# laurentbartholdi/SpaSM.jl

Measured on AMD Instinct MI355X. Metric: Schur nnz reduced/sec (GF(p) echelonize), 1Mx1M CSR, higher is better.
Workload: dtype int32 (GF(p) balanced residues); 1 GPU; BASELINE config 3: 1000000x1000000 CSR, 20 nnz/row, p=65521, seed 0x5A5A0003, Schur round 0; rows_per_gpu=1000000, npiv=169473, nnz_out=522630694, parallelism=single GPU

## Files before the change

### spasm.jl_amd/csrc/engine.hip

```cpp
#include "common.hpp"
#include "kernels.hpp"
#include "stream.hpp"
#include "wlevel.hpp"
#include "greedy.hpp"
#include "dense.hpp"
#include "spmv.hpp"
#include "spgemm.hpp"
#include "reshape.hpp"
#include "trsolve.hpp"
#include "batch.hpp"
#include "blocks.hpp"
#include "solve_batch.hpp"
#include "solver.hpp"
#include <cstring>
#include <rocprim/device/device_scan.hpp>
#include <rocprim/device/device_radix_sort.hpp>
#include <rocprim/device/device_segmented_radix_sort.hpp>
#include <vector>
#include <memory>
#include <stdexcept>
#include <type_traits>
#include <algorithm>
#include <cstring>
#include <cstdlib>
// ... 163 lines not shown
    default: break;
    }
}

template <int LOGT, int TPR, int WPB, int B, bool SMALL, int MINW = 1, int EPL = 1, int QX = 0, bool BLOOM = false, bool SEG = false> void launch_wstream(const StreamArgs &a, int nrows, int num_cu, size_t lds, hipStream_t s)
{
    static int per_cu_dev[kMaxDev] = {0};
    int &per_cu = per_cu_dev[current_device()];
    if (!per_cu) {
        HIPCHK(hipFuncSetAttribute((const void *)k_wstream<LOGT, TPR, WPB, B, SMALL, MINW, EPL, QX, BLOOM, SEG>, hipFuncAttributeMaxDynamicSharedMemorySize, (int)lds));
        int nb = 0;
        HIPCHK(hipOccupancyMaxActiveBlocksPerMultiprocessor(&nb, (const void *)k_wstream<LOGT, TPR, WPB, B, SMALL, MINW, EPL, QX, BLOOM, SEG>, WPB * 64, lds));
        per_cu = std::max(nb, 1);
    }
    if (nrows <= 0) return;
    const int rows_per_block = TPR == 64 ? WPB : 1;
    const int grid = std::max(1, std::min((nrows + rows_per_block - 1) / rows_per_block, num_cu * per_cu));
    hipLaunchKernelGGL((k_wstream<LOGT, TPR, WPB, B, SMALL, MINW, EPL, QX, BLOOM, SEG>), dim3(grid), dim3(WPB * 64), lds, s, a);
    HIPCHK(hipGetLastError());
}

inline bool stream_bloom()
{
    const char *e = getenv("SPASM_AMD_BLOOM");
    return e && atoi(e) != 0;
}
inline int stream_chunk_log()
{
    const char *e = getenv("SPASM_AMD_CHUNK");
    return e && atoi(e) == 128 ? 7 : 6;
}
enum StreamMode { STREAM_SEG = 0, STREAM_CHUNK64 = 1, STREAM_BLOOM = 2, STREAM_CHUNK128 = 3 };
inline StreamMode stream_mode(i64 buffer_entries)
{
    if (stream_chunk_log() == 7) return STREAM_CHUNK128;
    if (stream_bloom()) return STREAM_BLOOM;
    return buffer_entries < ((i64)1 << 29) ? STREAM_SEG : STREAM_CHUNK64;
}

const int kNumStreamClasses = 7;
inline int stream_logt(int c) { return 8 + c; }
inline int stream_tpr(int c) { return c <= 2 ? 64 : (c == 3 ? 128 : 256); }
inline int stream_wpb(int c) { return c == 3 ? 2 : 4; }
template <bool SMALL> void launch_stream_class(int cls, const StreamArgs &a, int nrows, int num_cu, size_t lds, hipStream_t s, StreamMode mode)
{
    if (mode == STREAM_SEG) {
        switch (cls) {
        case 0: launch_wstream<8, 64, 4, 4, SMALL, 1, 1, 0, false, true>(a, nrows, num_cu, lds, s); break;
        case 1: launch_wstream<9, 64, 4, 8, SMALL, 1, 1, 0, false, true>(a, nrows, num_cu, lds, s); break;
        case 2: launch_wstream<10, 64, 4, 8, SMALL, 1, 1, 0, false, true>(a, nrows, num_cu, lds, s); break;
        case 3: launch_wstream<11, 128, 2, 8, SMALL, 1, 1, 0, false, true>(a, nrows, num_cu, lds, s); break;
        case 4: launch_wstream<12, 256, 4, 8, SMALL, 1, 1, 0, false, true>(a, nrows, num_cu, lds, s); break;
        case 5: launch_wstream<13, 256, 4, 8, SMALL, 1, 1, 0, false, true>(a, nrows, num_cu, lds, s); break;
        case 6: launch_wstream<14, 256, 4, 8, SMALL, 1, 1, 0, false, true>(a, nrows, num_cu, lds, s); break;
        default: break;
        }
        return;
    }
    if (mode == STREAM_CHUNK128) {
        switch (cls) {
        case 0: launch_wstream<8, 64, 4, 2, SMALL, 1, 2>(a, nrows, num_cu, lds, s); break;
        case 1: launch_wstream<9, 64, 4, 4, SMALL, 1, 2>(a, nrows, num_cu, lds, s); break;
        case 2: launch_wstream<10, 64, 4, 4, SMALL, 1, 2>(a, nrows, num_cu, lds, s); break;
        case 3: launch_wstream<11, 128, 2, 4, SMALL, 1, 2>(a, nrows, num_cu, lds, s); break;
        case 4: launch_wstream<12, 256, 4, 4, SMALL, 1, 2>(a, nrows, num_cu, lds, s); break;
        case 5: launch_wstream<13, 256, 4, 4, SMALL, 1, 2>(a, nrows, num_cu, lds, s); break;
        case 6: launch_wstream<14, 256, 4, 4, SMALL, 1, 2>(a, nrows, num_cu, lds, s); break;
        default: break;
        }
        return;
    }
    if (mode == STREAM_BLOOM) {
        switch (cls) {
        case 0: launch_wstream<8, 64, 4, 4, SMALL, 1, 1, 0, true>(a, nrows, num_cu, lds, s); break;
        case 1: launch_wstream<9, 64, 4, 8, SMALL, 1, 1, 0, true>(a, nrows, num_cu, lds, s); break;
        case 2: launch_wstream<10, 64, 4, 8, SMALL, 1, 1, 0, true>(a, nrows, num_cu, lds, s); break;
        case 3: launch_wstream<11, 128, 2, 8, SMALL, 1, 1, 0, true>(a, nrows, num_cu, lds, s); break;
        case 4: launch_wstream<12, 256, 4, 8, SMALL, 1, 1, 0, true>(a, nrows, num_cu, lds, s); break;
        case 5: launch_wstream<13, 256, 4, 8, SMALL, 1, 1, 0, true>(a, nrows, num_cu, lds, s); break;
        case 6: launch_wstream<14, 256, 4, 8, SMALL, 1, 1, 0, true>(a, nrows, num_cu, lds, s); break;
        default: break;
        }
        return;
    }
    switch (cls) {
    case 0: launch_wstream<8, 64, 4, 4, SMALL>(a, nrows, num_cu, lds, s); break;
    case 1: launch_wstream<9, 64, 4, 8, SMALL>(a, nrows, num_cu, lds, s); break;
    case 2: launch_wstream<10, 64, 4, 8, SMALL>(a, nrows, num_cu, lds, s); break;
    case 3: launch_wstream<11, 128, 2, 8, SMALL>(a, nrows, num_cu, lds, s); break;
    case 4: launch_wstream<12, 256, 4, 8, SMALL>(a, nrows, num_cu, lds, s); break;
    case 5: launch_wstream<13, 256, 4, 8, SMALL>(a, nrows, num_cu, lds, s); break;
    case 6: launch_wstream<14, 256, 4, 8, SMALL>(a, nrows, num_cu, lds, s); break;
    default: break;
    }
}

struct Round {
    ZpField F;
    int m = 0;
    int num_cu = 256;
    hipStream_t stream = nullptr;
    Scanner scan;

    DevBuf<u64d> best;
    DevBuf<int> colflag, colscan, qinv_r, pivrow, pivcol, is_piv, rowflag, rowscan, np_rows;
    int npiv = 0, nnp = 0;
    DevBuf<i64d> ulen, uoff;
    i64 utotal = 0;
    DevBuf<int2> Ufull, UPP, UPN;
    DevBuf<UHdr> uhdr;
    bool use_uinv = false;
    DevMat E;
    DevBuf<int2> UinvPool;
    DevBuf<i64d> UinvStart, ubound;
    DevBuf<int> UinvLen;
    DevBuf<int4> colinfo;
    DevBuf<unsigned> pbits;
    DevBuf<i64d> rstart;
    DevBuf<int> rlen;
    i64 uinv_nnz = 0;
    DevBuf<int4> Lpool;
    DevBuf<int> Lidx;
    bool want_idx = false;
    DevBuf<int> sflag;
    DevBuf<int2> fixbuf;
    DevBuf<int> fixcnt;
    bool use_stream = true;
    StreamMode smode = STREAM_SEG;
    bool use_w = false;
    bool force_lists = false;
    DevBuf<int4> wcol;
    DevBuf<int2> wrow;
    DevBuf<int> wreject_list;
    i64 wtotal = 0;
    i64 wcap = 0;
    i64 w_entries = 0, w_long_rows = 0;
    i64 own_base = 0, wbase = 0;
    i64 own_total = 0;
    DevBuf<u64d> own_ctr;
    DevBuf<u64d> wstate, wblk;
    DevBuf<int> wmid_list, wbig_list, wbig_count;
    std::vector<int> wbig_at;
    bool want_w_row_stats = false;
    DevBuf<WLevRec> lev_recs;
    DevBuf<unsigned> lev0_sz, lev0_off;
    DevBuf<u64d> lev0_ent;
    i64 lev0_total = 0, lev0_entries = 0;
    int wave_per_cu_blocks = 0;
    DevBuf<int> lev, lev_keys, lev_iota, lev_order, lev_start_d, lev_flag;
    DevBuf<unsigned char> sort_tmp;
    std::vector<int> lev_start;
    int depth = -1;
    bool quiet_rejects = false;
    DevBuf<u64d> pool_ctr;
    int npool_active = NPOOL;
    u64d region_cap = 0;
    DevBuf<i64d> Lstart, bound, sstart;
    DevBuf<int> Llen, overflow_list, overflow2_list, fail_list;
    DevBuf<long long> pmask;
    int big_blocks = 0, big_npiv = -1;
    DevBuf<int> xdense;
    DevBuf<unsigned> bitmap;
    DevBuf<int4> bigscratch;
    DevBuf<RoundCounters> ctr;
    RoundCounters hctr;
    DevBuf<int> class_count, class_list;
    DevBuf<RowDesc> class_desc;
    int bigsc_blocks = 0, bigsc_m = -1;
    DevBuf<long long> sc_xdense;
    DevBuf<unsigned> sc_bitmap;
    DevBuf<int> sc_touched;
    DevBuf<u64d> stamps;
    DevMat S;
    i64 s_capacity = 0;
    i64 s_total_bound = 0;
    int free_cols = 0;
    hipEvent_t ev[5] = {nullptr, nullptr, nullptr, nullptr, nullptr};
    hipStream_t side = nullptr;
    hipStream_t twin_s[3] = {nullptr, nullptr, nullptr};
    hipEvent_t twin_ev[3] = {nullptr, nullptr, nullptr};
    hipEvent_t ev_fork = nullptr, ev_join = nullptr;
    hipStream_t lane_s[4] = {nullptr, nullptr, nullptr, nullptr};
    hipEvent_t lane_ev[4] = {nullptr, nullptr, nullptr, nullptr};
    hipEvent_t ev_cls_done[NHASHMAX] = {nullptr, nullptr, nullptr, nullptr, nullptr, nullptr, nullptr, nullptr};
    hipEvent_t ev_cls[NCLASS + 1];
    int launch_cls[NCLASS];
    int nlaunch = 0;
    int hclass_count[NCLASS];
    int nhash_used = 0;
    bool class_timing = true;

    Round()
    {
        memset(&hctr, 0, sizeof hctr);
        for (auto &e : ev) HIPCHK(hipEventCreate(&e));
        for (auto &e : ev_cls) { e = nullptr; HIPCHK(hipEventCreate(&e)); }
        memset(hclass_count, 0, sizeof hclass_count);
        memset(launch_cls, 0, sizeof launch_cls);
        if (const char *e = getenv("SPASM_AMD_STREAM")) use_stream = atoi(e) != 0;
        int dev = 0;
        hipDeviceProp_t prop;
        if (hipGetDevice(&dev) == hipSuccess && hipGetDeviceProperties(&prop, dev) == hipSuccess) num_cu = prop.multiProcessorCount;
    }
    ~Round()
    {
        for (auto &e : ev) if (e) (void)hipEventDestroy(e);
        for (auto &e : ev_cls) if (e) (void)hipEventDestroy(e);
        for (auto &e : ev_w) if (e) (void)hipEventDestroy(e);
        if (ev_fork) (void)hipEventDestroy(ev_fork);
        if (ev_join) (void)hipEventDestroy(ev_join);
        for (auto &e : lane_ev) if (e) (void)hipEventDestroy(e);
        for (auto &l : lane_s) if (l) (void)hipStreamDestroy(l);
        for (auto &e : ev_cls_done) if (e) (void)hipEventDestroy(e);
        if (side) (void)hipStreamDestroy(side);
        for (auto &e : twin_ev) if (e) (void)hipEventDestroy(e);
        for (auto &l : twin_s) if (l) (void)hipStreamDestroy(l);
    }

    void elect_local(const DevMat &A, int row_base, int row_stride = 1)
    {
        m = A.m;
        best.ensure((size_t)m + 1);
        hipLaunchKernelGGL(k_fill_u64, dim3(cdiv((i64)m + 1, 256)), dim3(256), 0, stream, (i64d)m + 1, (u64d)NO_BEST, best.p);
        HIPCHK(hipGetLastError());
        if (A.n > 0) {
            hipLaunchKernelGGL(k_elect, dim3(cdiv(A.n, 256)), dim3(256), 0, stream, A.n, row_base, row_stride, A.len.p, A.lead.p, best.p);
            HIPCHK(hipGetLastError());
        }
    }

    void assign_pivots()
    {
        colflag.ensure((size_t)m + 1);
        colscan.ensure((size_t)m + 1);
        qinv_r.ensure((size_t)m + 1);
        hipLaunchKernelGGL(k_col_flags, dim3(cdiv((i64)m + 1, 256)), dim3(256), 0, stream, m, best.p, colflag.p);
        HIPCHK(hipGetLastError());
        scan.exclusive(colflag.p, colscan.p, (size_t)m + 1, stream);
        HIPCHK(hipMemcpyAsync(&npiv, colscan.p + m, sizeof(int), hipMemcpyDeviceToHost, stream));
        HIPCHK(hipStreamSynchronize(stream));
        pivrow.ensure((size_t)npiv + 1);
        pivcol.ensure((size_t)npiv + 1);
        if (m > 0) {
            hipLaunchKernelGGL(k_col_assign, dim3(cdiv(m, 256)), dim3(256), 0, stream, m, best.p, colscan.p, qinv_r.p, pivrow.p, pivcol.p);
            HIPCHK(hipGetLastError());
        }
    }

    DevBuf<int> closed, colcnt, prop, newflag, newscan;
    bool quiet_fallbacks = false;
    bool quiet_known = false;
    DevBuf<int> pivval;
    bool want_pivval = false;
    DevBuf<u64d> best2;
    int n_leftmost = 0, n_open = 0;
    DevBuf<int> newpass, newidx, newrow_of_col, newrows;
    int open_count[OPEN_PASSES + 1] = {0};
    int open_nnew = 0, open_npass = 0;
    void open_begin(const DevMat &A, int row_base, int row_stride)
    {
        n_leftmost = npiv;
        n_open = 0;
        open_nnew = open_npass = 0;
        for (int &c : open_count) c = 0;
        closed.ensure((size_t)m + 1); colcnt.ensure((size_t)m + 1); newflag.ensure((size_t)m + 1); newscan.ensure((size_t)m + 1);
        newpass.ensure((size_t)m + 1); newidx.ensure((size_t)m + 1); newrow_of_col.ensure((size_t)m + 1); newrows.ensure((size_t)m + 1);
        best2.ensure((size_t)m + 1);
        prop.ensure((size_t)A.n + 1);
        is_piv.ensure((size_t)A.n + 1);
        HIPCHK(hipMemsetAsync(closed.p, 0, ((size_t)m + 1) * sizeof(int), stream));
        HIPCHK(hipMemsetAsync(newpass.p, 0, ((size_t)m + 1) * sizeof(int), stream));
        HIPCHK(hipMemsetAsync(is_piv.p, 0, ((size_t)A.n + 1) * sizeof(int), stream));
        if (npiv > 0) {
            hipLaunchKernelGGL(k_mark_rows, dim3(cdiv(npiv, 256)), dim3(256), 0, stream, npiv, row_base, row_stride, A.n, pivrow.p, is_piv.p);
            constexpr int TEAM = 8;
            hipLaunchKernelGGL((k_close_cols<TEAM>), dim3(cdiv((i64)npiv * TEAM, 256)), dim3(256), 0, stream, npiv, pivrow.p, row_base, row_stride, A.n, A.start.p, A.len.p,
                               A.ent.p, closed.p);
            HIPCHK(hipGetLastError());
        }
    }
    void open_hist(const DevMat &A)
    {
        HIPCHK(hipMemsetAsync(colcnt.p, 0, ((size_t)m + 1) * sizeof(int), stream));
        HIPCHK(hipMemsetAsync(newflag.p, 0, ((size_t)m + 1) * sizeof(int), stream));
        hipLaunchKernelGGL(k_fill_u64, dim3(cdiv((i64)m + 1, 256)), dim3(256), 0, stream, (i64d)m + 1, (u64d)NO_BEST, best2.p);
        if (A.n > 0) hipLaunchKernelGGL(k_col_histogram, dim3(cdiv((i64)A.n * 8, 256)), dim3(256), 0, stream, A.n, is_piv.p, A.start.p, A.len.p, A.ent.p, colcnt.p);
        HIPCHK(hipGetLastError());
    }
    void open_propose(const DevMat &A, int row_base, int row_stride)
    {
        constexpr int TEAM = 8;
        if (A.n > 0)
            hipLaunchKernelGGL((k_propose_open<TEAM>), dim3(cdiv((i64)A.n * TEAM, 256)), dim3(256), 0, stream, A.n, row_base, row_stride, is_piv.p, A.start.p, A.len.p,
                               A.ent.p, closed.p, colcnt.p, prop.p, best2.p);
        HIPCHK(hipGetLastError());
    }
    void open_accept(const DevMat &A, int row_base, int row_stride)
    {
        constexpr int TEAM = 8;
        if (A.n > 0)
            hipLaunchKernelGGL((k_accept_open<TEAM>), dim3(cdiv((i64)A.n * TEAM, 256)), dim3(256), 0, stream, A.n, row_base, row_stride, A.start.p, A.len.p, A.ent.p,
                               prop.p, best2.p, newflag.p);
        HIPCHK(hipGetLastError());
    }
    int open_record(const DevMat &A, int pass, int row_base, int row_stride)
    {
        scan.exclusive(newflag.p, newscan.p, (size_t)m + 1, stream);
        int nacc = 0;
        HIPCHK(hipMemcpyAsync(&nacc, newscan.p + m, sizeof(int), hipMemcpyDeviceToHost, stream));
        HIPCHK(hipStreamSynchronize(stream));
        if (nacc == 0) return 0;
        constexpr int TEAM = 8;
        hipLaunchKernelGGL(k_record_open, dim3(cdiv(m, 256)), dim3(256), 0, stream, m, pass, newflag.p, newscan.p, best2.p, newpass.p, newidx.p,
                           newrow_of_col.p, newrows.p, is_piv.p, row_base, row_stride, A.n);
        hipLaunchKernelGGL((k_close_cols<TEAM>), dim3(cdiv((i64)nacc * TEAM, 256)), dim3(256), 0, stream, nacc, newrows.p, row_base, row_stride, A.n, A.start.p, A.len.p,
                           A.ent.p, closed.p);
        HIPCHK(hipGetLastError());
        open_count[pass] = nacc;
        open_nnew += nacc;
        open_npass = pass;
        return nacc;
    }
    int open_finish()
    {
        const int nnew = open_nnew;
        if (nnew == 0) return 0;
        int base[OPEN_PASSES + 2] = {0};
        for (int pass = open_npass, at = 0; pass >= 1; pass--) { base[pass] = at; at += open_count[pass]; }
        static_assert(OPEN_PASSES == 4, "k_col_assign2 takes the bases of four passes");
        pivrow.ensure((size_t)npiv + nnew + 1);
        pivcol.ensure((size_t)npiv + nnew + 1);
        hipLaunchKernelGGL(k_col_assign2, dim3(cdiv(m, 256)), dim3(256), 0, stream, m, nnew, make_int4(base[1], base[2], base[3], base[4]), best.p, newpass.p,
                           newidx.p, newrow_of_col.p, colscan.p, qinv_r.p, pivrow.p, pivcol.p);
        HIPCHK(hipGetLastError());
        npiv += nnew;
        n_open = nnew;
        return nnew;
    }
    int extend_pivots_on_open_columns(const DevMat &A)
    {
        n_leftmost = npiv;
        n_open = 0;
        if (npiv == 0 || A.n == 0) return 0;
        open_begin(A, 0, 1);
        for (int pass = 1; pass <= OPEN_PASSES; pass++) {
            open_hist(A);
            open_propose(A, 0, 1);
            open_accept(A, 0, 1);
            if (open_record(A, pass, 0, 1) == 0) break;
        }
        return open_finish();
    }

    DevBuf<int> gr_accept, gr_ascan, gr_lev, gr_iota, gr_order, gr_prow, gr_pcol, gr_flag;
    DevBuf<u64d> gr_keys, gr_keys2;
    int n_greedy = 0;
    int extend_pivots_cycle_free(const DevMat &A)
    {
        n_greedy = 0;
        if (npiv == 0 || A.n == 0) return 0;
        const int n = A.n;
        best2.ensure((size_t)m + 1);
        prop.ensure((size_t)n + 1);
        gr_accept.ensure((size_t)n + 1);
        gr_ascan.ensure((size_t)n + 1);
        is_piv.ensure((size_t)n + 1);
        HIPCHK(hipMemsetAsync(is_piv.p, 0, ((size_t)n + 1) * sizeof(int), stream));
        hipLaunchKernelGGL(k_mark_rows, dim3(cdiv(npiv, 256)), dim3(256), 0, stream, npiv, 0, 1, n, pivrow.p, is_piv.p);
        HIPCHK(hipGetLastError());
// ... 434 lines not shown
        a.F = F;
        a.list_stride = npiv;
        auto launch_wg = [&](int tier, int grid) {
            a.tslots = tier ? big_slots : wl_mid_slots();
            a.blk_base = num_cu * 16 * 4 + (tier ? num_cu * 8 : 0);
            if (tier) {
                if (F.small) hipLaunchKernelGGL((k_wlevel_wg<true, NT_BIG>), dim3(grid), dim3(NT_BIG), lds_big, stream, a);
                else hipLaunchKernelGGL((k_wlevel_wg<false, NT_BIG>), dim3(grid), dim3(NT_BIG), lds_big, stream, a);
            } else {
                if (F.small) hipLaunchKernelGGL((k_wlevel_wg<true, NT_MID>), dim3(grid), dim3(NT_MID), lds_mid, stream, a);
                else hipLaunchKernelGGL((k_wlevel_wg<false, NT_MID>), dim3(grid), dim3(NT_MID), lds_mid, stream, a);
            }
        };
        {
            const int cnt0 = lev_start[1];
            hipLaunchKernelGGL(k_wlevel0, dim3(std::max(1, std::min(cdiv((i64)cnt0 * 16, 256), num_cu * 8))), dim3(256), 0, stream, cnt0, lev_recs.p, lev0_off.p,
                               UPN.p, wrow.p, wcol.p, (unsigned)wbase, F);
        }
        for (int L = 1; L <= depth; L++) {
            const int cnt = lev_start[(size_t)L + 1] - lev_start[(size_t)L];
            if (cnt <= 0) continue;
            int *const mid_count = wbig_count.p + (size_t)(2 * L) * WL_NSUB * WL_SUBSTRIDE, *const big_count = wbig_count.p + (size_t)(2 * L + 1) * WL_NSUB * WL_SUBSTRIDE;
            const int known_mid = -1, known_big = -1;
            a.cnt = cnt;
            a.rec_base = lev_start[(size_t)L];
            a.mid_list = wmid_list.p;
            a.mid_count = mid_count;
            a.big_list = wbig_list.p;
            a.big_count = big_count;
            a.list = nullptr;
            a.count = nullptr;
            if (cnt > 2048) {
                a.recs = lev_recs.p + lev_start[(size_t)L];
                a.tslots = 0;
                a.blk_base = 0;
                const int grid = std::min(cdiv(cnt, 4), num_cu * wave_per_cu_blocks);
                if (F.small) hipLaunchKernelGGL(k_wlevel_wave<true>, dim3(grid), dim3(256), 0, stream, a);
                else hipLaunchKernelGGL(k_wlevel_wave<false>, dim3(grid), dim3(256), 0, stream, a);
                a.recs = lev_recs.p;
                if (known_mid != 0) {
                    a.list = wmid_list.p;
                    a.count = mid_count;
                    a.big_list = nullptr;
                    launch_wg(0, known_mid < 0 ? num_cu * mid_per_cu : std::min(num_cu * mid_per_cu, known_mid));
                }
            } else {
                a.recs = lev_recs.p;
                if (cnt <= num_cu) {
                    a.big_list = nullptr;
                    launch_wg(1, cnt);
                    continue;
                }
                launch_wg(0, std::min(num_cu * mid_per_cu, cnt));
            }
            if (known_big != 0) {
                a.list = wbig_list.p;
                a.count = big_count;
                a.big_list = nullptr;
                launch_wg(1, known_big < 0 ? num_cu : std::min(num_cu, known_big));
            }
        }
        HIPCHK(hipGetLastError());
        HIPCHK(hipEventRecord(ev_w[1], stream));
    }

    void prepare_w_(i64 expected_rows, i64 own_entries)
    {
        use_w = false;
        wtotal = 0;
        ms_levels = 0;
        ms_w_sizing = 0;
        if (!use_stream || force_lists || want_idx || m >= (1 << 24) || npiv == 0 || expected_rows < 2 * (i64)npiv) return;
        {
            HIPCHK(hipStreamSynchronize(stream));
            const double t0 = spasm_wtime();
            build_levels();
            HIPCHK(hipStreamSynchronize(stream));
            ms_levels = 1e3 * (spasm_wtime() - t0);
        }
        if (depth < 0) return;
        const double t_sizing0 = spasm_wtime();
        const i64 own_room = ((own_entries + own_entries / 2 + (i64)num_cu * 16 * 16 * 256 + NPOOL) + 15) & ~(i64)15;
        own_base = (utotal + 15) & ~(i64)15;
        wbase = own_base + own_room;
        i64 cap = std::min<i64>(64 * std::max<i64>(utotal, 1 << 16), (i64)0xffffffffLL - wbase - 64);
        {
            size_t fr = 0, totmem = 0;
            HIPCHK(hipMemGetInfo(&fr, &totmem));
            const i64 have = (i64)UPN.n;
            const i64 room = have + (i64)(fr / 2 / sizeof(int2));
            if (wbase + cap + 1 > room) cap = room - wbase - 1;
        }
        cap &= ~(i64)15;
        if (cap < 4 * std::max<i64>(utotal, 1 << 12) || cap < 2 * lev0_total) return;
        if ((i64)UPN.n < wbase + cap + 1) {
            DevBuf<int2> both;
            both.alloc((size_t)(wbase + cap) + 1);
            if (utotal > 0) HIPCHK(hipMemcpyAsync(both.p, UPN.p, (size_t)utotal * sizeof(int2), hipMemcpyDeviceToDevice, stream));
            HIPCHK(hipStreamSynchronize(stream));
            UPN = std::move(both);
        }
        wcap = cap;
        wrow.ensure((size_t)npiv + 1);
        wcol.ensure((size_t)m + 1);
        wmid_list.ensure((size_t)WL_NSUB * (size_t)npiv + 1);
        wbig_list.ensure((size_t)WL_NSUB * (size_t)npiv + 1);
        wbig_count.ensure((size_t)2 * (WMAXLEV + 2) * WL_NSUB * WL_SUBSTRIDE);
        wstate.ensure(WS_WORDS);
        wblk.ensure((size_t)2 * wblk_slots());
        own_ctr.ensure((size_t)NPOOL * POOL_STRIDE);
        pbits.ensure((size_t)cdiv(m, 256) * 8 + 2);
        hipLaunchKernelGGL(k_pbits, dim3(cdiv(m, 256)), dim3(256), 0, stream, m, qinv_r.p, pbits.p);
        HIPCHK(hipGetLastError());
        wbig_at.assign((size_t)2 * (depth + 2), 0);
        {
            HIPCHK(hipStreamSynchronize(stream));
            ms_w_sizing = 1e3 * (spasm_wtime() - t_sizing0);
        }
        build_w_levels();
        hipLaunchKernelGGL(k_wstats, dim3(cdiv(npiv, 256)), dim3(256), 0, stream, npiv, wrow.p, wstate.p);
        HIPCHK(hipGetLastError());
        u64d ws[WS_WORDS];
        HIPCHK(hipMemcpyAsync(ws, wstate.p, sizeof ws, hipMemcpyDeviceToHost, stream));
        const bool wdebug = getenv("SPASM_AMD_WDEBUG") != nullptr || want_w_row_stats;
        std::vector<int> parts;
        if (wdebug) {
            parts.resize((size_t)2 * (depth + 1) * WL_NSUB * WL_SUBSTRIDE);
            HIPCHK(hipMemcpyAsync(parts.data(), wbig_count.p, parts.size() * sizeof(int), hipMemcpyDeviceToHost, stream));
        }
        HIPCHK(hipStreamSynchronize(stream));
        if (wdebug)
            for (int k = 0; k < 2 * (depth + 1); k++)
                for (int sb = 0; sb < WL_NSUB; sb++) wbig_at[(size_t)k] += parts[((size_t)k * WL_NSUB + sb) * WL_SUBSTRIDE];
        if (ws[WS_ERROR]) throw EngineError("a hash table of the W build filled up (internal bound violated)");
        if (getenv("SPASM_AMD_WDEBUG")) {
            fprintf(stderr, "[wlevel] npiv %d depth %d entries %llu cursor %llu unavailable %llu long rows %llu; rows per level (medium, large):", npiv, depth,
                    (unsigned long long)ws[WS_ENTRIES], (unsigned long long)ws[WS_CURSOR], (unsigned long long)ws[WS_UNAVAIL], (unsigned long long)ws[WS_BIGROWS]);
            for (int L = 0; L <= depth; L++)
                fprintf(stderr, " %d (%d, %d)", lev_start[(size_t)L + 1] - lev_start[(size_t)L], wbig_at[(size_t)2 * L], wbig_at[(size_t)2 * L + 1]);
            fprintf(stderr, "\n");
        }
        if (ws[WS_UNAVAIL] * 64 > (u64d)npiv) return;
        wtotal = (i64)std::min<u64d>(ws[WS_CURSOR], (u64d)cap);
        w_entries = (i64)ws[WS_ENTRIES] + lev0_entries;
        w_long_rows = 0;
        for (int k = 0; k < 2 * (depth + 1); k++) w_long_rows += wbig_at[(size_t)k];
        own_total = own_room;
        use_w = true;
    }

    void run_solve(const DevMat &M, const int *rows, const int *self_idx, int nrows)
    {
        const bool wmode = use_w && !force_lists && !self_idx && !want_idx;
        {
            static_assert(sizeof(RoundCounters) % 4 == 0, "cleared word by word");
            const int nctr_words = (int)(NCTR * sizeof(RoundCounters) / 4), npool_words = NPOOL * POOL_STRIDE;
            const int span = std::max(std::max(nctr_words, npool_words), nrows + 1);
            if (wmode) own_ctr.ensure((size_t)NPOOL * POOL_STRIDE);
            hipLaunchKernelGGL(k_solve_reset, dim3(cdiv(span, 256)), dim3(256), 0, stream, nrows, (unsigned *)ctr.p, nctr_words, pool_ctr.p,
                               npool_words, class_count.p, (int)NCLASS, bound.p, pmask.p, sflag.p, wmode ? own_ctr.p : (u64d *)nullptr);
            HIPCHK(hipGetLastError());
        }
        if (nrows == 0) return;
        SolveArgs a;
        a.nrows = nrows;
        a.rows = rows;
        a.self_idx = self_idx;
        a.retry = nullptr;
        a.retry_count = nullptr;
        a.start = M.start.p;
        a.len = M.len.p;
        a.ent = M.ent.p;
        a.qinv_r = qinv_r.p;
        a.uhdr = uhdr.p;
        a.UPP = UPP.p;
        a.Lpool = Lpool.p;
        a.Lidx = want_idx ? Lidx.p : nullptr;
        a.Lpool2 = nullptr;
        a.lpool_cap = region_cap;
        a.pool_ctr = pool_ctr.p;
        a.npool = npool_active;
        a.Lstart = Lstart.p;
        a.Llen = Llen.p;
        a.bound = bound.p;
        a.free_cols = free_cols;
        a.overflow_list = overflow_list.p;
        a.overflow_count = &ctr.p->solve_overflow;
        a.ctr = ctr.p;
        a.F = F;
        if (!wmode && !use_uinv) {
            launch_chain(a, nrows, true);
            return;
        }
        rstart.ensure((size_t)nrows + 1);
        rlen.ensure((size_t)nrows + 1);
        hipLaunchKernelGGL(k_gather_rows, dim3(cdiv(nrows, 256)), dim3(256), 0, stream, nrows, rows, M.start.p, M.len.p, rstart.p, rlen.p);
        HIPCHK(hipGetLastError());
        if (wmode) {
            wreject_list.ensure((size_t)nrows + 1);
            WPlanArgs wp;
            wp.nrows = nrows;
            wp.rstart = rstart.p;
            wp.rlen = rlen.p;
            wp.ent = M.ent.p;
            wp.pbits = pbits.p;
            wp.wcol = wcol.p;
            wp.Lpool = Lpool.p;
            wp.lpool_cap = region_cap;
            wp.pool_ctr = pool_ctr.p;
            wp.npool = npool_active;
            wp.upn = UPN.p;
            wp.own_base = (unsigned)own_base;
            wp.own_cap = (u64d)own_total / (u64d)npool_active;
            wp.own_ctr = own_ctr.p;
            wp.Lstart = Lstart.p;
            wp.Llen = Llen.p;
            wp.bound = bound.p;
            wp.pmask = pmask.p;
            wp.sflag = sflag.p;
            wp.free_cols = free_cols;
            wp.max_bound = (int)kClasses[kNumStreamClasses - 1].cap;
            wp.wave_row_bound = (int)kClasses[2].cap;
            wp.overflow_list = wreject_list.p;
            wp.overflow_count = &ctr.p->wplan_reject;
            wp.ctr = ctr.p;
            wp.F = F;
            smode = stream_mode(wbase + wcap);
            wp.chunk_log = smode == STREAM_CHUNK128 ? 7 : 6;
            constexpr int TEAM = 16, TPB = 256;
            const dim3 grid(std::min(cdiv((i64)nrows * TEAM, TPB), num_cu * 16));
            if (smode == STREAM_SEG) hipLaunchKernelGGL((k_wplan<TEAM, TPB, true>), grid, dim3(TPB), 0, stream, wp);
            else hipLaunchKernelGGL((k_wplan<TEAM, TPB, false>), grid, dim3(TPB), 0, stream, wp);
            HIPCHK(hipGetLastError());
            if (!use_uinv) {
                if (!quiet_rejects) launch_chain(a, nrows, true, wreject_list.p, &ctr.p->wplan_reject);
                return;
            }
        }
        CombineArgs c;
        c.nrows = nrows;
        c.self_idx = self_idx;
        c.rstart = rstart.p;
        c.rlen = rlen.p;
        c.ent = M.ent.p;
        c.colinfo = colinfo.p;
        c.pbits = pbits.p;
        c.uhdr = uhdr.p;
        c.UinvPool = UinvPool.p;
        c.Lpool = Lpool.p;
        c.Lidx = want_idx ? Lidx.p : nullptr;
        c.sflag = nullptr;
        c.lpool_cap = region_cap;
        c.pool_ctr = pool_ctr.p;
        c.npool = npool_active;
        c.Lstart = Lstart.p;
        c.Llen = Llen.p;
        c.bound = bound.p;
        c.pmask = pmask.p;
        c.free_cols = free_cols;
        c.retry = wmode ? wreject_list.p : nullptr;
        c.retry_count = wmode ? &ctr.p->wplan_reject : nullptr;
        c.overflow_list = overflow2_list.p;
        c.overflow_count = &ctr.p->combine_overflow;
        c.ctr = ctr.p;
        {
            const char *dbg = getenv("SPASM_DBG");
            c.dbg = dbg ? atoi(dbg) : 0;
        }
        c.F = F;
        {
            constexpr int TEAM = 16, LOGC = 8, TPB = 256;
            const int grid = std::min(cdiv((i64)nrows * TEAM, TPB), num_cu * 8);
            if (F.small) hipLaunchKernelGGL((k_combine<TEAM, LOGC, TPB, true>), dim3(grid), dim3(TPB), 0, stream, c);
            else hipLaunchKernelGGL((k_combine<TEAM, LOGC, TPB, false>), dim3(grid), dim3(TPB), 0, stream, c);
            HIPCHK(hipGetLastError());
        }
        if (!quiet_fallbacks) {
            c.retry = overflow2_list.p;
            c.retry_count = &ctr.p->combine_overflow;
            c.overflow_list = overflow_list.p;
            c.overflow_count = &ctr.p->solve_overflow;
            {
                constexpr int TEAM = 64, LOGC = 12, TPB = 64;
                const int grid = std::min(nrows, num_cu * 4);
                if (F.small) hipLaunchKernelGGL((k_combine<TEAM, LOGC, TPB, true>), dim3(grid), dim3(TPB), 0, stream, c);
                else hipLaunchKernelGGL((k_combine<TEAM, LOGC, TPB, false>), dim3(grid), dim3(TPB), 0, stream, c);
                HIPCHK(hipGetLastError());
            }
            launch_chain(a, nrows, false);
        }
    }

    RoundCounters read_counters(int total_bound_of = -1)
    {
        std::vector<RoundCounters> h(NCTR);
        i64d tot = 0;
        HIPCHK(hipMemcpyAsync(h.data(), ctr.p, NCTR * sizeof(RoundCounters), hipMemcpyDeviceToHost, stream));
        if (total_bound_of >= 0) HIPCHK(hipMemcpyAsync(&tot, sstart.p + total_bound_of, sizeof(i64d), hipMemcpyDeviceToHost, stream));
        HIPCHK(hipStreamSynchronize(stream));
        if (total_bound_of >= 0) s_total_bound = tot;
        RoundCounters c = h[0];
        for (int i = 1; i < NCTR; i++) {
            c.applications += h[i].applications;
            c.nnz_reduced += h[i].nnz_reduced;
            c.segments += h[i].segments;
            c.lpool_overflow += h[i].lpool_overflow;
            c.scatter_overflow += h[i].scatter_overflow;
            c.nonempty_out += h[i].nonempty_out;
            c.nnz_out += h[i].nnz_out;
            c.stream_redo += h[i].stream_redo;
            c.stream_fix += h[i].stream_fix;
            for (int k = 0; k < 16; k++) { c.class_ent[k] += h[i].class_ent[k]; c.class_seg[k] += h[i].class_seg[k]; }
        }
        return c;
    }

    u64d pool_used()
    {
        std::vector<u64d> h((size_t)NPOOL * POOL_STRIDE);
        HIPCHK(hipMemcpyAsync(h.data(), pool_ctr.p, h.size() * sizeof(u64d), hipMemcpyDeviceToHost, stream));
        HIPCHK(hipStreamSynchronize(stream));
        u64d mx = 0;
        for (int r = 0; r < npool_active; r++) mx = std::max(mx, h[(size_t)r * POOL_STRIDE]);
        return mx * (u64d)npool_active;
    }

    i64 solve_phase(const DevMat &M, const int *rows, const int *self_idx, int nrows, i64 lpool_guess, i64 max_pool = ((i64)1 << 62))
    {
        i64 pool = std::min<i64>(std::max<i64>(lpool_guess, 1 << 16), max_pool);
        for (;;) {
            alloc_solve(nrows, pool);
            run_solve(M, rows, self_idx, nrows);
            run_bounds(nrows);
            const RoundCounters c = read_counters(nrows);
            const i64 tot = s_total_bound;
            if (c.lpool_overflow) {
                if (pool >= max_pool) return -1;
                pool = std::min<i64>(std::max<i64>(pool * 2, (i64)(pool_used() * 5 / 4) + 1024), max_pool);
                continue;
            }
            return tot;
        }
    }

    void run_bounds(int nrows)
    {
        scan.exclusive(bound.p, sstart.p, (size_t)nrows + 1, stream);
    }

    i64 fetch_total_bound(int nrows)
    {
        i64d tot = 0;
        HIPCHK(hipMemcpyAsync(&tot, sstart.p + nrows, sizeof(i64d), hipMemcpyDeviceToHost, stream));
        HIPCHK(hipStreamSynchronize(stream));
        s_total_bound = tot;
        return tot;
    }

    static int n_lanes() { static const int v = [] { const char *e = getenv("SPASM_AMD_STREAM_LANES"); return std::min(4, std::max(1, e ? atoi(e) : 2)); }(); return v; }
    static int n_twins() { static const int v = [] { const char *e = getenv("SPASM_AMD_TWIN_STREAMS"); return std::min(4, std::max(1, e ? atoi(e) : 2)); }(); return v; }
    void ensure_streams()
    {
        if (!side) {
            HIPCHK(hipStreamCreateWithFlags(&side, hipStreamNonBlocking));
            HIPCHK(hipEventCreateWithFlags(&ev_fork, hipEventDisableTiming));
            HIPCHK(hipEventCreateWithFlags(&ev_join, hipEventDisableTiming));
        }
        if (!ev_cls_done[0]) for (auto &e : ev_cls_done) HIPCHK(hipEventCreateWithFlags(&e, hipEventDisableTiming));
        for (int l = 1; l < n_lanes(); l++)
            if (!lane_s[l]) {
                HIPCHK(hipStreamCreateWithFlags(&lane_s[l], hipStreamNonBlocking));
                HIPCHK(hipEventCreateWithFlags(&lane_ev[l], hipEventDisableTiming));
            }
        for (int t = 0; t < n_twins() - 1; t++)
            if (!twin_s[t]) {
                HIPCHK(hipStreamCreateWithFlags(&twin_s[t], hipStreamNonBlocking));
                HIPCHK(hipEventCreateWithFlags(&twin_ev[t], hipEventDisableTiming));
            }
    }
    void ensure_big_scatter(hipStream_t s)
    {
        if (bigsc_m == m) return;
        const i64 per = std::max<i64>((i64)m, 1) * 13;
        bigsc_blocks = (int)std::max<i64>(1, std::min<i64>((i64)num_cu * 8, ((i64)2 << 30) / per));
        bigsc_m = m;
        const size_t nw = ((size_t)std::max(m, 1) + 31) / 32;
        sc_xdense.alloc((size_t)bigsc_blocks * (size_t)std::max(m, 1));
        sc_bitmap.alloc((size_t)bigsc_blocks * nw);
        sc_touched.alloc((size_t)bigsc_blocks * (size_t)std::max(m, 1));
        sc_xdense.zero(s);
        sc_bitmap.zero(s);
    }
    void warm_scatter()
    {
        ensure_streams();
        ensure_big_scatter(stream);
        ScatterArgs a;
        memset(&a, 0, sizeof a);
        StreamArgs sa;
        memset(&sa, 0, sizeof sa);
        const int nhash = F.small ? kNumHashClasses : kNumHashClasses - 1;
        for (int c = 0; c < nhash; c++) {
            const size_t lds = scatter_lds_bytes(kClasses[c], F.small);
            if (F.small) launch_scatter_class<true>(c, a, 0, lds, stream);
            else launch_scatter_class<false>(c, a, 0, lds, stream);
        }
        for (int c = 0; c < std::min(nhash, kNumStreamClasses); c++) {
            const size_t lds = stream_lds_bytes(stream_logt(c), stream_tpr(c), stream_wpb(c));
            const StreamMode mode = stream_mode(use_w ? wbase + wcap : 0);
            if (F.small) launch_stream_class<true>(c, sa, 0, num_cu, lds, stream, mode);
            else launch_stream_class<false>(c, sa, 0, num_cu, lds, stream, mode);
        }
    }

    void run_scatter(const DevMat &M, const int *rows, int nrows)
    {
        const int4 *recs = Lpool.p;
        S.n = nrows;
        S.m = m;
        nlaunch = 0;
        if (nrows == 0) return;
        int nhash = F.small ? kNumHashClasses : kNumHashClasses - 1;
        const bool streaming = use_w && !force_lists && !want_idx;
        BinArgs b;
        b.nrows = nrows;
        b.bound = bound.p;
        b.Llen = Llen.p;
        for (int c = 0; c < NCLASS; c++) b.cap[c] = -1;
        for (int c = 0; c < nhash; c++) b.cap[c] = kClasses[c].cap;
        b.lazy_terms = zp_lazy_terms(F);
        b.class_count = class_count.p;
        b.class_list = class_list.p;
        b.rows = rows;
        b.start = M.start.p;
        b.len = M.len.p;
        b.orig = M.orig.p;
        b.Lstart = Lstart.p;
        b.sstart = sstart.p;
        b.pmask = pmask.p;
        b.sflag = sflag.p;
        b.stream_classes = streaming ? std::min(nhash, kNumStreamClasses) : 0;
        b.Sorig = S.orig.p;
        b.fixcnt = fixcnt.p;
        b.desc = class_desc.p;
        hipLaunchKernelGGL(k_bin, dim3(cdiv(nrows, 1024)), dim3(256), 0, stream, b);
        HIPCHK(hipGetLastError());

        ScatterArgs a;
        a.ent = M.ent.p;
        a.qinv_r = qinv_r.p;
        a.uhdr = uhdr.p;
        a.UPN = UPN.p;
        a.Lpool = recs;
        a.Sent = S.ent.p;
        a.Slen = S.len.p;
        a.Slead = S.lead.p;
        a.ctr = ctr.p;
        a.F = F;
        {
            const char *dbg = getenv("SPASM_DBG");
            a.dbg = dbg ? atoi(dbg) : 0;
        }
        a.stamps = nullptr;
#ifdef SPASM_STAMPS
        stamps.ensure(NCLASS * 2 * NSTAMP);
        HIPCHK(hipMemsetAsync(stamps.p, 0, NCLASS * 2 * NSTAMP * sizeof(u64d), stream));
        a.stamps = stamps.p;
#endif
        StreamArgs sa;
        sa.ent = M.ent.p;
        sa.qinv_r = qinv_r.p;
        sa.UPN = UPN.p;
        sa.Lpool = recs;
        sa.Sent = S.ent.p;
        sa.Slen = S.len.p;
        sa.Slead = S.lead.p;
        sa.ctr = ctr.p;
        sa.F = F;
        sa.dbg = a.dbg;
        sa.stamps = a.stamps;
        sa.fixbuf = fixbuf.p;
        sa.fixcnt = fixcnt.p;
        nhash_used = nhash;
        const int first_side = 6;
        const bool use_side = !class_timing && (nhash > first_side || streaming);
        if (use_side) {
            ensure_streams();
            HIPCHK(hipEventRecord(ev_fork, stream));
            HIPCHK(hipStreamWaitEvent(side, ev_fork, 0));
        }
        auto mark = [&](int cls_id, hipStream_t s) {
            if (!class_timing || nlaunch >= NCLASS) return;
            HIPCHK(hipEventRecord(ev_cls[nlaunch], s));
            launch_cls[nlaunch++] = cls_id;
        };
        auto launch_class = [&](int c, hipStream_t s) {
            mark(c, s);
            a.cls = c;
            a.class_count = class_count.p + c;
            a.desc = class_desc.p + (size_t)c * nrows;
            const size_t lds = scatter_lds_bytes(kClasses[c], F.small);
            int per_cu = (int)std::min<size_t>(32 / kClasses[c].wpb, (160 * 1024) / lds);
            if (per_cu < 1) per_cu = 1;
            const int rows_per_block = kClasses[c].tpr == 64 ? kClasses[c].wpb : 1;
            const int grid = std::max(1, std::min(cdiv(nrows, rows_per_block), num_cu * per_cu));
            if (F.small) launch_scatter_class<true>(c, a, grid, lds, s);
            else launch_scatter_class<false>(c, a, grid, lds, s);
        };
        auto launch_stream_cls = [&](int c, hipStream_t s) {
            if (!streaming || c >= kNumStreamClasses) return;
            mark(NSTREAM0 + c, s);
            sa.cls = NSTREAM0 + c;
            sa.class_count = class_count.p + NSTREAM0 + c;
            sa.desc = class_desc.p + (size_t)(NSTREAM0 + c) * nrows;
            sa.redo_count = class_count.p + c;
            sa.redo_desc = class_desc.p + (size_t)c * nrows;
            const size_t lds = stream_lds_bytes(stream_logt(c), stream_tpr(c), stream_wpb(c));
            if (F.small) launch_stream_class<true>(c, sa, nrows, num_cu, lds, s, smode);
            else launch_stream_class<false>(c, sa, nrows, num_cu, lds, s, smode);
        };
        auto launch_stream_fix = [&](hipStream_t s) {
            if (!streaming) return;
            mark(NCLASS - 1, s);
            StreamFixArgs fa;
            fa.nrows = nrows;
            fa.fixcnt = fixcnt.p;
            fa.fixbuf = fixbuf.p;
            fa.sstart = sstart.p;
            fa.Sent = S.ent.p;
            fa.Slen = S.len.p;
            fa.Slead = S.lead.p;
            fa.ctr = ctr.p;
            fa.F = F;
            hipLaunchKernelGGL(k_stream_fix, dim3(cdiv(nrows, 64)), dim3(256), 0, s, fa);
            HIPCHK(hipGetLastError());
        };
        auto launch_big = [&](hipStream_t s) {
            ensure_big_scatter(s);
            mark(NHASHMAX - 1, s);
            BigScatterArgs bb;
            bb.s = a;
            bb.s.cls = NHASHMAX - 1;
            bb.s.class_count = class_count.p + (NHASHMAX - 1);
            bb.s.desc = class_desc.p + (size_t)(NHASHMAX - 1) * nrows;
            bb.m = std::max(m, 1);
            bb.nwords = (std::max(m, 1) + 31) / 32;
            bb.xdense = sc_xdense.p;
            bb.bitmap = sc_bitmap.p;
            bb.touched = sc_touched.p;
            hipLaunchKernelGGL(k_scatter_big, dim3(bigsc_blocks), dim3(256), 0, s, bb);
            HIPCHK(hipGetLastError());
        };
        if (use_side && streaming) {
            const int lanes = n_lanes();
            for (int l = 1; l < lanes; l++) HIPCHK(hipStreamWaitEvent(lane_s[l], ev_fork, 0));
            const int ntwin = n_twins();
            for (int c = nhash - 1; c >= 0; c--) {
                const int l = (nhash - 1 - c) % lanes;
                hipStream_t lane = l ? lane_s[l] : stream;
                launch_stream_cls(c, lane);
                HIPCHK(hipEventRecord(ev_cls_done[c], lane));
                const int t = (nhash - 1 - c) % ntwin;
                hipStream_t tw = t ? twin_s[t - 1] : side;
                HIPCHK(hipStreamWaitEvent(tw, ev_cls_done[c], 0));
                launch_class(c, tw);
            }
            for (int l = 1; l < lanes; l++) {
                HIPCHK(hipEventRecord(lane_ev[l], lane_s[l]));
                HIPCHK(hipStreamWaitEvent(stream, lane_ev[l], 0));
            }
            for (int t = 0; t < ntwin - 1; t++) {
                HIPCHK(hipEventRecord(twin_ev[t], twin_s[t]));
                HIPCHK(hipStreamWaitEvent(stream, twin_ev[t], 0));
            }
            launch_stream_fix(stream);
            launch_big(side);
            HIPCHK(hipEventRecord(ev_join, side));
            HIPCHK(hipStreamWaitEvent(stream, ev_join, 0));
        } else if (use_side) {
            for (int c = nhash - 1; c >= first_side; c--) launch_class(c, side);
            launch_big(side);
            HIPCHK(hipEventRecord(ev_join, side));
            for (int c = 0; c < first_side; c++) launch_class(c, stream);
            HIPCHK(hipStreamWaitEvent(stream, ev_join, 0));
        } else {
            for (int c = nhash - 1; c >= 0; c--) launch_stream_cls(c, stream);
            launch_stream_fix(stream);
            for (int c = 0; c < nhash; c++) launch_class(c, stream);
            launch_big(stream);
            if (class_timing) HIPCHK(hipEventRecord(ev_cls[nlaunch], stream));
        }
        hipLaunchKernelGGL(k_scatter_mark_failed, dim3(cdiv(nrows, 256)), dim3(256), 0, stream, nrows, Llen.p, S.len.p, S.lead.p);
        HIPCHK(hipGetLastError());
        HIPCHK(hipMemcpyAsync(S.start.p, sstart.p, ((size_t)nrows + 1) * sizeof(i64d), hipMemcpyDeviceToDevice, stream));
    }

    void fetch_counters()
    {
        hctr = read_counters();
        int *cc = hclass_count;
        HIPCHK(hipMemcpyAsync(cc, class_count.p, NCLASS * sizeof(int), hipMemcpyDeviceToHost, stream));
        HIPCHK(hipStreamSynchronize(stream));
#ifdef SPASM_STAMPS
        {
            std::vector<u64d> h(NCLASS * 2 * NSTAMP);
            HIPCHK(hipMemcpy(h.data(), stamps.p, h.size() * sizeof(u64d), hipMemcpyDeviceToHost));
            static const char *names[NSTAMP] = {"prologue", "issue", "wait-loads", "own", "rounds", "remainder", "sweep", "-"};
            static const char *snames[NSTAMP] = {"top+own", "chunks", "next-req", "rowend", "reset", "rotate", "-", "-"};
            for (int c = NSTREAM0; c < NCLASS; c++) {
                const double waves = (double)h[(size_t)c * 2 * NSTAMP + NSTAMP];
                if (waves == 0) continue;
                fprintf(stderr, "[stamps] stream class %d rows %d waves %.0f: cycles per wave:", c - NSTREAM0, cc[c], waves);
                for (int i = 0; i < 6; i++) fprintf(stderr, " %s=%.0f", snames[i], (double)h[(size_t)c * 2 * NSTAMP + i] / waves);
                fprintf(stderr, "\n");
            }
            for (int c = 0; c < NHASHMAX; c++) {
                const double waves = (double)h[(size_t)c * 2 * NSTAMP + NSTAMP];
                if (waves == 0) continue;
                fprintf(stderr, "[stamps] class %d rows %d waves %.0f: cycles per wave:", c, cc[c], waves);
                for (int i = 0; i < 7; i++) fprintf(stderr, " %s=%.0f", names[i], (double)h[(size_t)c * 2 * NSTAMP + i] / waves);
                fprintf(stderr, "\n");
            }
        }
#endif
        if (hctr.lpool_overflow) throw EngineError("multiplier pool exhausted");
        if (hctr.scatter_overflow) throw EngineError("a hash table of the scatter kernel filled up (internal bound violated)");
    }
};

void upload_csr_strided(const struct spasm_csr *A, int row_lo, int row_hi, int stride, DevMat &M, hipStream_t s);

void upload_csr(const struct spasm_csr *A, int row_lo, int row_hi, DevMat &M, hipStream_t s)
{
    const int n = row_hi - row_lo;
    const i64 base = A->p[row_lo];
    const i64 nnz = A->p[row_hi] - base;
    M.n = n;
    M.m = A->m;
    M.start.ensure((size_t)n + 1);
    M.len.ensure((size_t)n + 1);
    M.lead.ensure((size_t)n + 1);
    M.orig.ensure((size_t)n + 1);
    M.ent.ensure((size_t)nnz + 1);
    DevBuf<i64d> dp;
    DevBuf<int> dj, dx;
    dp.alloc((size_t)n + 1);
    dj.alloc((size_t)nnz + 1);
    dx.alloc((size_t)nnz + 1);
    std::vector<i64d> hp((size_t)n + 1);
    for (int i = 0; i <= n; i++) hp[(size_t)i] = A->p[row_lo + i] - base;
    HIPCHK(hipMemcpyAsync(dp.p, hp.data(), ((size_t)n + 1) * sizeof(i64d), hipMemcpyHostToDevice, s));
    if (nnz > 0) {
        HIPCHK(hipMemcpyAsync(dj.p, A->j + base, (size_t)nnz * sizeof(int), hipMemcpyHostToDevice, s));
        if (A->x) HIPCHK(hipMemcpyAsync(dx.p, A->x + base, (size_t)nnz * sizeof(int), hipMemcpyHostToDevice, s));
        hipLaunchKernelGGL(k_pack_entries, dim3(std::min<i64>(cdiv(nnz, 256), 65536)), dim3(256), 0, s, (i64d)nnz, zp_field_make(A->field->p), dj.p,
                           A->x ? dx.p : nullptr, M.ent.p);
        HIPCHK(hipGetLastError());
    }
    if (n > 0) {
        hipLaunchKernelGGL(k_pack_rows, dim3(cdiv(n, 256)), dim3(256), 0, s, n, row_lo, 1, dp.p, M.start.p, M.len.p, M.orig.p);
        HIPCHK(hipGetLastError());
        constexpr int TEAM = 8;
        if (A->x) hipLaunchKernelGGL((k_drop_zeros<TEAM>), dim3(cdiv((i64)n * TEAM, 256)), dim3(256), 0, s, n, M.start.p, M.len.p, M.ent.p);
        hipLaunchKernelGGL((k_row_lead<TEAM>), dim3(cdiv((i64)n * TEAM, 256)), dim3(256), 0, s, n, M.start.p, M.len.p, M.ent.p, M.lead.p);
        HIPCHK(hipGetLastError());
    }
    HIPCHK(hipStreamSynchronize(s));
}

void upload_csr_strided(const struct spasm_csr *A, int row_lo, int row_hi, int stride, DevMat &M, hipStream_t s)
{
    if (stride <= 1) { upload_csr(A, row_lo, row_hi, M, s); return; }
    const int n = row_hi > row_lo ? (row_hi - row_lo + stride - 1) / stride : 0;
    std::vector<i64d> hp((size_t)n + 1, 0);
    for (int i = 0; i < n; i++) { const int g = row_lo + i * stride; hp[(size_t)i + 1] = hp[(size_t)i] + (A->p[g + 1] - A->p[g]); }
    const i64 nnz = hp[(size_t)n];
    std::vector<int> hj((size_t)nnz + 1), hx((size_t)nnz + 1);
    for (int i = 0; i < n; i++) {
        const int g = row_lo + i * stride;
        const i64 len = A->p[g + 1] - A->p[g];
        memcpy(hj.data() + hp[(size_t)i], A->j + A->p[g], sizeof(int) * (size_t)len);
        if (A->x) memcpy(hx.data() + hp[(size_t)i], A->x + A->p[g], sizeof(int) * (size_t)len);
    }
    M.n = n;
    M.m = A->m;
    M.start.ensure((size_t)n + 1);
    M.len.ensure((size_t)n + 1);
    M.lead.ensure((size_t)n + 1);
    M.orig.ensure((size_t)n + 1);
    M.ent.ensure((size_t)nnz + 1);
    DevBuf<i64d> dp;
    DevBuf<int> dj, dx;
    dp.alloc((size_t)n + 1);
    dj.alloc((size_t)nnz + 1);
    dx.alloc((size_t)nnz + 1);
    HIPCHK(hipMemcpyAsync(dp.p, hp.data(), ((size_t)n + 1) * sizeof(i64d), hipMemcpyHostToDevice, s));
    if (nnz > 0) {
        HIPCHK(hipMemcpyAsync(dj.p, hj.data(), (size_t)nnz * sizeof(int), hipMemcpyHostToDevice, s));
        if (A->x) HIPCHK(hipMemcpyAsync(dx.p, hx.data(), (size_t)nnz * sizeof(int), hipMemcpyHostToDevice, s));
        hipLaunchKernelGGL(k_pack_entries, dim3(std::min<i64>(cdiv(nnz, 256), 65536)), dim3(256), 0, s, (i64d)nnz, zp_field_make(A->field->p), dj.p,
                           A->x ? dx.p : nullptr, M.ent.p);
        HIPCHK(hipGetLastError());
    }
    if (n > 0) {
        hipLaunchKernelGGL(k_pack_rows, dim3(cdiv(n, 256)), dim3(256), 0, s, n, row_lo, stride, dp.p, M.start.p, M.len.p, M.orig.p);
        HIPCHK(hipGetLastError());
        constexpr int TEAM = 8;
        if (A->x) hipLaunchKernelGGL((k_drop_zeros<TEAM>), dim3(cdiv((i64)n * TEAM, 256)), dim3(256), 0, s, n, M.start.p, M.len.p, M.ent.p);
        hipLaunchKernelGGL((k_row_lead<TEAM>), dim3(cdiv((i64)n * TEAM, 256)), dim3(256), 0, s, n, M.start.p, M.len.p, M.ent.p, M.lead.p);
        HIPCHK(hipGetLastError());
    }
    HIPCHK(hipStreamSynchronize(s));
}

void require_device()
{
    int n = 0;
    hipError_t e = hipGetDeviceCount(&n);
    if (e != hipSuccess || n <= 0) throw EngineError("no HIP device: the MI355X engine has no CPU fallback");
}

void check_input(const struct spasm_csr *A, const char *who)
{
    if (!A) throw EngineError(std::string(who) + ": NULL matrix");
    const i64 p = A->field->p;
    if (p <= 2 || p > 0xfffffffbLL) throw EngineError(std::string(who) + ": prime out of range (2 < p <= 0xfffffffb)");
    if (!A->x && A->p[A->n] > 0) throw EngineError(std::string(who) + ": matrix without values");
}

thread_local std::vector<spasm_amd_round_stats> g_last_rounds;
thread_local int g_multi_finish = 0;
thread_local i64 g_dense_stats[8] = {0, 0, 0, 0, 0, 0, 0, 0};
inline void dense_stats_note(int kind, int R, int C, int block)
{
    g_dense_stats[0]++;
    g_dense_stats[1] = kind; g_dense_stats[2] = R; g_dense_stats[3] = C; g_dense_stats[4] = block;
}

i64 read_bytes_of(const RoundCounters &c, int m) { return 8 * (i64)c.nnz_reduced + 16 * (i64)c.segments + 4 * (i64)m; }

void fill_stats(spasm_amd_round_stats &st, const Round &R, int round, int rows_in, i64 nnz_in)
// ... 9531 lines not shown
```

Measured before the change: 190.9 billion nnz/s.

## Funnel streaming redo rows into one class and skip empty direct class launches

Result: slower. 184.8 billion nnz/s (-3.2%).

```diff
diff --git a/spasm.jl_amd/csrc/engine.hip b/spasm.jl_amd/csrc/engine.hip
--- a/spasm.jl_amd/csrc/engine.hip
+++ b/spasm.jl_amd/csrc/engine.hip
@@ -339,6 +339,8 @@
     std::vector<int> lev_start;
     int depth = -1;
     bool quiet_rejects = false;
+    bool solve_wmode = false;
+    int solve_rejects = -1;
     DevBuf<u64d> pool_ctr;
     int npool_active = NPOOL;
     u64d region_cap = 0;
@@ -364,12 +366,9 @@
     int free_cols = 0;
     hipEvent_t ev[5] = {nullptr, nullptr, nullptr, nullptr, nullptr};
     hipStream_t side = nullptr;
-    hipStream_t twin_s[3] = {nullptr, nullptr, nullptr};
-    hipEvent_t twin_ev[3] = {nullptr, nullptr, nullptr};
     hipEvent_t ev_fork = nullptr, ev_join = nullptr;
     hipStream_t lane_s[4] = {nullptr, nullptr, nullptr, nullptr};
     hipEvent_t lane_ev[4] = {nullptr, nullptr, nullptr, nullptr};
-    hipEvent_t ev_cls_done[NHASHMAX] = {nullptr, nullptr, nullptr, nullptr, nullptr, nullptr, nullptr, nullptr};
     hipEvent_t ev_cls[NCLASS + 1];
     int launch_cls[NCLASS];
     int nlaunch = 0;
@@ -398,10 +397,7 @@
         if (ev_join) (void)hipEventDestroy(ev_join);
         for (auto &e : lane_ev) if (e) (void)hipEventDestroy(e);
         for (auto &l : lane_s) if (l) (void)hipStreamDestroy(l);
-        for (auto &e : ev_cls_done) if (e) (void)hipEventDestroy(e);
         if (side) (void)hipStreamDestroy(side);
-        for (auto &e : twin_ev) if (e) (void)hipEventDestroy(e);
-        for (auto &l : twin_s) if (l) (void)hipStreamDestroy(l);
     }
 
     void elect_local(const DevMat &A, int row_base, int row_stride = 1)
@@ -1142,6 +1138,8 @@
     void run_solve(const DevMat &M, const int *rows, const int *self_idx, int nrows)
     {
         const bool wmode = use_w && !force_lists && !self_idx && !want_idx;
+        solve_wmode = wmode;
+        solve_rejects = -1;
         {
             static_assert(sizeof(RoundCounters) % 4 == 0, "cleared word by word");
             const int nctr_words = (int)(NCTR * sizeof(RoundCounters) / 4), npool_words = NPOOL * POOL_STRIDE;
@@ -1324,6 +1322,7 @@
             run_bounds(nrows);
             const RoundCounters c = read_counters(nrows);
             const i64 tot = s_total_bound;
+            solve_rejects = c.wplan_reject;
             if (c.lpool_overflow) {
                 if (pool >= max_pool) return -1;
                 pool = std::min<i64>(std::max<i64>(pool * 2, (i64)(pool_used() * 5 / 4) + 1024), max_pool);
@@ -1348,24 +1347,18 @@
     }
 
     static int n_lanes() { static const int v = [] { const char *e = getenv("SPASM_AMD_STREAM_LANES"); return std::min(4, std::max(1, e ? atoi(e) : 2)); }(); return v; }
-    static int n_twins() { static const int v = [] { const char *e = getenv("SPASM_AMD_TWIN_STREAMS"); return std::min(4, std::max(1, e ? atoi(e) : 2)); }(); return v; }
     void ensure_streams()
     {
         if (!side) {
             HIPCHK(hipStreamCreateWithFlags(&side, hipStreamNonBlocking));
             HIPCHK(hipEventCreateWithFlags(&ev_fork, hipEventDisableTiming));
             HIPCHK(hipEventCreateWithFlags(&ev_join, hipEventDisableTiming));
-        }
-        if (!ev_cls_done[0]) for (auto &e : ev_cls_done) HIPCHK(hipEventCreateWithFlags(&e, hipEventDisableTiming));
+            HIPCHK(hipEventCreateWithFlags(&lane_ev[0], hipEventDisableTiming));
+        }
         for (int l = 1; l < n_lanes(); l++)
             if (!lane_s[l]) {
                 HIPCHK(hipStreamCreateWithFlags(&lane_s[l], hipStreamNonBlocking));
                 HIPCHK(hipEventCreateWithFlags(&lane_ev[l], hipEventDisableTiming));
-            }
-        for (int t = 0; t < n_twins() - 1; t++)
-            if (!twin_s[t]) {
-                HIPCHK(hipStreamCreateWithFlags(&twin_s[t], hipStreamNonBlocking));
-                HIPCHK(hipEventCreateWithFlags(&twin_ev[t], hipEventDisableTiming));
             }
     }
     void ensure_big_scatter(hipStream_t s)
@@ -1497,14 +1490,16 @@
             if (F.small) launch_scatter_class<true>(c, a, grid, lds, s);
             else launch_scatter_class<false>(c, a, grid, lds, s);
         };
+        const int redo_cls = nhash - 1;
+        const bool no_direct_rows = streaming && solve_wmode && (quiet_known ? quiet_rejects : solve_rejects == 0);
         auto launch_stream_cls = [&](int c, hipStream_t s) {
             if (!streaming || c >= kNumStreamClasses) return;
             mark(NSTREAM0 + c, s);
             sa.cls = NSTREAM0 + c;
             sa.class_count = class_count.p + NSTREAM0 + c;
             sa.desc = class_desc.p + (size_t)(NSTREAM0 + c) * nrows;
-            sa.redo_count = class_count.p + c;
-            sa.redo_desc = class_desc.p + (size_t)c * nrows;
+            sa.redo_count = class_count.p + redo_cls;
+            sa.redo_desc = class_desc.p + (size_t)redo_cls * nrows;
             const size_t lds = stream_lds_bytes(stream_logt(c), stream_tpr(c), stream_wpb(c));
             if (F.small) launch_stream_class<true>(c, sa, nrows, num_cu, lds, s, smode);
             else launch_stream_class<false>(c, sa, nrows, num_cu, lds, s, smode);
@@ -1544,26 +1539,20 @@
         if (use_side && streaming) {
             const int lanes = n_lanes();
             for (int l = 1; l < lanes; l++) HIPCHK(hipStreamWaitEvent(lane_s[l], ev_fork, 0));
-            const int ntwin = n_twins();
+            if (!no_direct_rows) for (int c = redo_cls - 1; c >= 0; c--) launch_class(c, side);
             for (int c = nhash - 1; c >= 0; c--) {
                 const int l = (nhash - 1 - c) % lanes;
-                hipStream_t lane = l ? lane_s[l] : stream;
-                launch_stream_cls(c, lane);
-                HIPCHK(hipEventRecord(ev_cls_done[c], lane));
-                const int t = (nhash - 1 - c) % ntwin;
-                hipStream_t tw = t ? twin_s[t - 1] : side;
-                HIPCHK(hipStreamWaitEvent(tw, ev_cls_done[c], 0));
-                launch_class(c, tw);
+                launch_stream_cls(c, l ? lane_s[l] : stream);
             }
+            HIPCHK(hipEventRecord(lane_ev[0], stream));
+            HIPCHK(hipStreamWaitEvent(side, lane_ev[0], 0));
             for (int l = 1; l < lanes; l++) {
                 HIPCHK(hipEventRecord(lane_ev[l], lane_s[l]));
+                HIPCHK(hipStreamWaitEvent(side, lane_ev[l], 0));
                 HIPCHK(hipStreamWaitEvent(stream, lane_ev[l], 0));
             }
-            for (int t = 0; t < ntwin - 1; t++) {
-                HIPCHK(hipEventRecord(twin_ev[t], twin_s[t]));
-                HIPCHK(hipStreamWaitEvent(stream, twin_ev[t], 0));
-            }
             launch_stream_fix(stream);
+            launch_class(redo_cls, side);
             launch_big(side);
             HIPCHK(hipEventRecord(ev_join, side));
             HIPCHK(hipStreamWaitEvent(stream, ev_join, 0));
@@ -1576,7 +1565,8 @@
         } else {
             for (int c = nhash - 1; c >= 0; c--) launch_stream_cls(c, stream);
             launch_stream_fix(stream);
-            for (int c = 0; c < nhash; c++) launch_class(c, stream);
+            for (int c = 0; c < nhash; c++)
+                if (c == redo_cls || !no_direct_rows) launch_class(c, stream);
             launch_big(stream);
             if (class_timing) HIPCHK(hipEventRecord(ev_cls[nlaunch], stream));
         }
```
